# Robotics-Engineer-khy/ti5_isaacgym

Measured on AMD Instinct MI355X. Metric: env-steps/sec at 8192 envs, t1_dh_stand, 1/2/4/8 MI355X; obs/reward parity, higher is better.
Workload: dtype f32

## Files before the change

### ti5_isaacgym_amd/csrc/t1env_device.h

```cpp
#pragma once
#include <hip/hip_runtime.h>

#include "../../include/t1env.h"
#include "t1_dynamics.h"

namespace t1 {

struct DevWriter {
  float* rootp;
  float* rigidp;
  float* contactp;
  __device__ void root(const float* v) {
#pragma unroll
    for (int i = 0; i < 13; ++i) rootp[i] = v[i];
  }
  __device__ void rigid(int b, const float* v) {
#pragma unroll
    for (int i = 0; i < 13; ++i) rigidp[b * 13 + i] = v[i];
  }
  __device__ void contact(int b, V3<float> f) {
    contactp[b * 3 + 0] = f.x;
    contactp[b * 3 + 1] = f.y;
    contactp[b * 3 + 2] = f.z;
  }
// ... 349 lines not shown
        store16B<SC1>(out0 + i, o);
        continue;
      }
      const uint32_t ow[4] = {o.x, o.y, o.z, o.w};
#pragma unroll
      for (int k = 0; k < 8; ++k) {
        const uint32_t e = i + k;
        if (e >= lim) break;
        if (e - (e / ROW) * ROW < ROW - F) store2B<SC1>(out0 + e, (uint16_t)(ow[k / 2] >> (16 * (k & 1))));
      }
    }
  }
}

__device__ __forceinline__ void shift_history(const ShiftArgs& S, int64_t t0, int64_t stride) {
  if (S.half) {
    shift_range_h<T1_NOBS, T1_HIST>(reinterpret_cast<const uint16_t*>(S.obs_in), reinterpret_cast<uint16_t*>(S.obs_out),
                                    S.total_obs, 0, (S.total_obs + 7) / 8, t0, stride);
    shift_range_h<T1_NPRIV, T1_CHIST>(reinterpret_cast<const uint16_t*>(S.priv_in),
                                      reinterpret_cast<uint16_t*>(S.priv_out), S.total_priv, 0, (S.total_priv + 7) / 8,
                                      t0, stride);
    return;
  }
  shift_range<T1_NOBS, T1_HIST>(S.obs_in, S.obs_out, S.total_obs, 0, (S.total_obs + 3) / 4, t0, stride);
  shift_range<T1_NPRIV, T1_CHIST>(S.priv_in, S.priv_out, S.total_priv, 0, (S.total_priv + 3) / 4, t0, stride);
}

template <int U = SHIFT_UNROLL>
__device__ __forceinline__ void shift_rows_range_sc1(const ShiftArgs& S, int64_t r0, int64_t r1, int64_t t0,
                                                 int64_t stride) {
  if (S.half) {
    shift_rows_f16<T1_NOBS, T1_HIST, true, U>(reinterpret_cast<const uint16_t*>(S.obs_in),
                                              reinterpret_cast<uint16_t*>(S.obs_out), S.total_obs, r0, r1, (int)t0,
                                              (int)stride);
    shift_rows_f16<T1_NPRIV, T1_CHIST, true, U>(reinterpret_cast<const uint16_t*>(S.priv_in),
                                                reinterpret_cast<uint16_t*>(S.priv_out), S.total_priv, r0, r1, (int)t0,
                                                (int)stride);
    return;
  }
  shift_rows_f32<T1_NOBS, T1_HIST, true, U>(S.obs_in, S.obs_out, S.total_obs, r0, r1, (int)t0, (int)stride);
  shift_rows_f32<T1_NPRIV, T1_CHIST, true, U>(S.priv_in, S.priv_out, S.total_priv, r0, r1, (int)t0, (int)stride);
}

__device__ __forceinline__ void zero_hist(float* buf, bool half, int64_t row, int width, int count, int t0, int stride) {
  if (half) {
    uint16_t* o = reinterpret_cast<uint16_t*>(buf) + row * width;
    for (int c = t0; c < count; c += stride) o[c] = 0;
  } else {
    float* o = buf + row * width;
    for (int c = t0; c < count; c += stride) o[c] = 0.0f;
  }
}

__device__ __forceinline__ void zero_history_row(const ShiftArgs& S, int64_t row, int t0, int stride) {
  zero_hist(S.obs_out, S.half, row, T1_NOBS * T1_HIST, T1_NOBS * (T1_HIST - 1), t0, stride);
  zero_hist(S.priv_out, S.half, row, T1_NPRIV * T1_CHIST, T1_NPRIV * (T1_CHIST - 1), t0, stride);
}

}
```

### ti5_isaacgym_amd/csrc/t1env_dyn6.hip

```cpp
#include <hip/hip_runtime.h>

#define T1_CONTACT_ONE_COPY

#ifdef T1_PROBE_SIMD
__device__ unsigned g_t1_simd6[4096][8];
#endif
#ifdef T1_PROBE_CLOCK
__device__ unsigned long long g_t1_clock6[4];
constexpr int T1_WGSUM6_N = 4 + 6;
__device__ unsigned long long g_t1_wgtime6[4096][4];
__device__ unsigned long long g_t1_wgsum6[4096][T1_WGSUM6_N];
#define T1_CLOCK_WAIT_BEGIN() const unsigned long long t1c_w0 = __builtin_amdgcn_s_memtime();
#define T1_CLOCK_SHIFT_END(wi)                                                     \
  if ((threadIdx.x & 63) == 0 && blockIdx.x < 4096 && (wi) >= 0)                   \
    atomicAdd(&g_t1_wgsum6[blockIdx.x][4 + (wi)], __builtin_amdgcn_s_memtime() - t1c_w0);
#define T1_CLOCK_LOOP_END()                                                        \
  if (threadIdx.x == 0 && blockIdx.x < 4096) g_t1_wgtime6[blockIdx.x][3] = __builtin_amdgcn_s_memrealtime();
#define T1_CLOCK_WAIT_END(k)                                                       \
  if (threadIdx.x == 0 && blockIdx.x < 4096)                                       \
    atomicAdd(&g_t1_wgsum6[blockIdx.x][k], __builtin_amdgcn_s_memtime() - t1c_w0);
#define T1_CLOCK_BEGIN()                                                           \
  unsigned long long t1c_cyc0 = 0, t1c_rt0 = 0;                                    \
  if (threadIdx.x == 0) {                                                          \
    t1c_cyc0 = __builtin_amdgcn_s_memtime();                                       \
    t1c_rt0 = __builtin_amdgcn_s_memrealtime();                                    \
    if (blockIdx.x < 4096) { g_t1_wgtime6[blockIdx.x][0] = t1c_rt0; g_t1_wgtime6[blockIdx.x][2] = 0; } \
  }
#define T1_CLOCK_END()                                                             \
  if (threadIdx.x == 0) {                                                          \
    const unsigned long long c1 = __builtin_amdgcn_s_memtime(), r1 = __builtin_amdgcn_s_memrealtime(); \
    atomicAdd(&g_t1_clock6[0], c1 - t1c_cyc0);                                     \
    atomicAdd(&g_t1_clock6[1], r1 - t1c_rt0);                                      \
    atomicAdd(&g_t1_clock6[2], 1ull);                                              \
    if (blockIdx.x < 4096) {                                                       \
      g_t1_wgtime6[blockIdx.x][1] = r1;                                            \
      atomicAdd(&g_t1_wgsum6[blockIdx.x][0], c1 - t1c_cyc0);                       \
    }                                                                              \
  }                                                                                \
  T1_CLOCK_WAVE_END();
#define T1_CLOCK_WAVE_END()                                                        \
  if ((threadIdx.x & 63) == 0 && blockIdx.x < 4096)                                \
    atomicMax(&g_t1_wgtime6[blockIdx.x][2], (unsigned long long)__builtin_amdgcn_s_memrealtime());
#else
#define T1_CLOCK_BEGIN() ((void)0)
#define T1_CLOCK_END() ((void)0)
#define T1_CLOCK_WAVE_END() ((void)0)
#define T1_CLOCK_WAIT_BEGIN() ((void)0)
#define T1_CLOCK_WAIT_END(k) ((void)0)
#define T1_CLOCK_SHIFT_END(wi) ((void)0)
#define T1_CLOCK_LOOP_END() ((void)0)
#endif

#define T1_PROF_WAVES 8
#define T1_PROF_NAME(x) x##6
#include "t1env_prof.h"

#include "t1_dyn5.h"
#include "t1env_device.h"
#include "t1env_internal.h"
#include "t1env_postphys.h"
#include "t1env_fused.h"
#include "t1env_roles.h"

using namespace t1;

constexpr int NE6 = 32;
constexpr int D6_BLOCK = 512;

enum : int { WB_TAU = 0, WB_AC = 8, WB_R = 29, WB_N = 35 };
struct SubspaceRows { float4 r[NLEG][2][64]; };
enum : int { R_RG = 0, R_G = 6, R_N = 12 };
enum : int { WC_SHA = 0, WC_SHB = 1, WC_FTA = 2, WC_FTB = 3, WC_SSH = 4, WC_SFT = 5, WC_N = 6 };
constexpr int SHIFT6_MASK = (1 << 1) | (1 << 5) | (1 << 2) | (1 << 6) | (1 << 3) | (1 << 7);
__device__ __forceinline__ int role_of(int wave) { return (int)((0x76543210u >> (4 * wave)) & 0xFu); }
constexpr int SHIFT6_WAVES = __builtin_popcount(SHIFT6_MASK);
static_assert((SHIFT6_MASK & 0x11) == 0, "W0 / W4 (the core chain's SIMD) do not shift");

struct Dyn6Lds {
  DynModel model;
  Rows4<Q_N> st;
  Rows4<WB_N> wb;
  SubspaceRows sj;
  Rows4<R_N> w1;
  Rows4<XCH> wc[WC_N];
  PdStage<64> pd;
  float cap[CAP5_N][64];
  float act[12][NE6];
  float epi[EPI_N][NE6];
  float fr[FR_N][NE6];
  float vish[64];
  float vift[64];
  float amx[4][64];
  LegParams<float> pl[64];
  BaseParams<float> pb[64];
  float rtf[2][3][64];
  float rsf[2][3][64];
};
T1_ROWS_ALIGNED(Dyn6Lds, st);
T1_ROWS_ALIGNED(Dyn6Lds, wb);
T1_ROWS_ALIGNED(Dyn6Lds, sj);
T1_ROWS_ALIGNED(Dyn6Lds, w1);
T1_ROWS_ALIGNED(Dyn6Lds, wc);
static_assert(sizeof(Rows4<XCH>) % 16 == 0 && alignof(Dyn6Lds) % 16 == 0, "every wc[i], and the struct itself");

template <int F, int H, bool HALF>
__device__ __forceinline__ void shift_chunk_elems(const uint8_t* in0, uint8_t* out0, uint32_t i, uint32_t nel) {
  constexpr uint32_t ROW = F * H, PER = HALF ? 8 : 4;
#pragma unroll 1
  for (uint32_t k = 0; k < PER; ++k) {
    const uint32_t e = i + k;
    if (e < nel && e % ROW < ROW - F) {
      if constexpr (HALF)
        reinterpret_cast<uint16_t*>(out0)[e] = reinterpret_cast<const uint16_t*>(in0)[e + F];
      else
        reinterpret_cast<float*>(out0)[e] = reinterpret_cast<const float*>(in0)[e + F];
    }
  }
}
template <int F, int H, bool HALF>
__device__ __forceinline__ void shp_range(int64_t total, int64_t r0, int64_t r1, int sl, int nsl, uint32_t& lo,
                                          uint32_t& hi, uint32_t& lim, uint32_t& nel) {
  constexpr uint32_t ROW = F * H, PER = HALF ? 8 : 4;
  lim = (uint32_t)(total - r0 * (int64_t)ROW);
  const uint32_t span = (uint32_t)((r1 - r0) * ROW);
  nel = span < lim ? span : lim;
  const uint32_t n = (nel + PER - 1) / PER;
  lo = n * (uint32_t)sl / (uint32_t)nsl;
  hi = n * (uint32_t)(sl + 1) / (uint32_t)nsl;
}
typedef float shift_f4 __attribute__((ext_vector_type(4), aligned(2)));
template <int F, bool HALF, int U>
__device__ __forceinline__ void shift_loads(const uint8_t* in0, uint32_t lo, uint32_t lim, int t0, int stride,
                                            float4* a) {
  constexpr uint32_t PER = HALF ? 8 : 4, ES = HALF ? 2 : 4;
#pragma unroll
  for (int u = 0; u < U; ++u) {
    const uint32_t src = (lo + (uint32_t)(t0 + u * stride)) * PER + F;
    const uint32_t sc = src + PER <= lim ? src : lim - PER;
    const shift_f4 v = *reinterpret_cast<const shift_f4*>(in0 + (size_t)sc * ES);
    a[u] = make_float4(v.x, v.y, v.z, v.w);
  }
}
template <int F, int H, bool HALF, int U>
__device__ __forceinline__ void shift_stores(const uint8_t* in0, uint8_t* out0, uint32_t lo, uint32_t hi,
                                             uint32_t lim, uint32_t nel, int t0, int stride, const float4* a) {
  constexpr uint32_t PER = HALF ? 8 : 4, ES = HALF ? 2 : 4;
  uint32_t slow = 0;
#pragma unroll
  for (int u = 0; u < U; ++u) {
// ... 644 lines not shown
          }
        } else {
          const int s = role == 2 ? 0 : 1;
          const int b = s == 0 ? bsh : bft;
          const float vt = restitution_target(M, eg, s == 0 ? lds.vish[lane] : lds.vift[lane]);
          const V3<float> f = body_contact_force(M, T, b, Ko[s].Rb, Ko[s].p, F.abs, Ko[s].V, mu, vt);
          lds.rtf[s][0][lane] = f.x; lds.rtf[s][1][lane] = f.y; lds.rtf[s][2][lane] = f.z;
        }
      }
      T1_PROF_MARK(10);
      if (role == 6) {
        const int s_dof = (nsub - 1) - B.dof_lag_timestep[n] % 10;
        const int s_imu = (nsub - 1) - B.imu_lag_timestep[n] % 10;
        BaseState<float> sb;
        float q[NLEG], qd[NLEG];
        read_state_rows(lds.st, lane, sb, q, qd);
        record_substep(M, lds.pb[lane], LG, lds, nsub - 1, s_dof, s_imu, N, n, j0, leg, lane, active, sb, q, qd);
        if (active) {
          float* const dof_dst = B.dof_hist + ((size_t)n * 4 + (ctr & 3u)) * 24;
          float* const imu_dst = B.imu_hist + ((size_t)n * 2 + (ctr & 1u)) * 8;
          if (s_dof < nsub) {
#pragma unroll
            for (int k = 0; k < NLEG; ++k) {
              dof_dst[j0 + k] = lds.cap[k][lane];
              dof_dst[12 + j0 + k] = lds.cap[NLEG + k][lane];
            }
          }
          if (leg == 0 && s_imu < nsub) {
            const float quat[4] = {lds.cap[2 * NLEG][lane], lds.cap[2 * NLEG + 1][lane], lds.cap[2 * NLEG + 2][lane],
                                   lds.cap[2 * NLEG + 3][lane]};
            const float w[3] = {lds.cap[2 * NLEG + 4][lane], lds.cap[2 * NLEG + 5][lane], lds.cap[2 * NLEG + 6][lane]};
            capture_imu(quat, w, imu_dst);
          }
        }
      }
      __syncthreads();
      T1_PROF_MARK(11);
      if (role == 6) {
        float* cf = B.contact_forces + (size_t)n * 39;
#pragma unroll
        for (int s = 0; s < 2; ++s) {
          const int b = s == 0 ? bsh : bft;
          const float f[3] = {lds.rtf[s][0][lane] + lds.rsf[s][0][lane], lds.rtf[s][1][lane] + lds.rsf[s][1][lane],
                              lds.rtf[s][2][lane] + lds.rsf[s][2][lane]};
          if (active) { cf[b * 3 + 0] = f[0]; cf[b * 3 + 1] = f[1]; cf[b * 3 + 2] = f[2]; }
          if (FUSED && s == 1) {
            const int r = leg == 0 ? F_C0 : F_C1;
            lds.fr[r][e] = f[0]; lds.fr[r + 1][e] = f[1]; lds.fr[r + 2][e] = f[2];
          }
        }
      }
    }
    if constexpr (FUSED) {
      __syncthreads();
      T1_PROF_MARK(12);
      if (role == 1)
        fused_epilogue_staged<POST_A_STATE, NE6, true>(M, C, B, A, S, FA, dyn_blocks, lane, lds.epi, lds.fr, lds.act,
                                                       lds.act + NLEG);
      else if (role == 2)
        fused_epilogue_obs<POST_OBS_PRIV, NE6>(M, C, B, A, lane, lds.epi, lds.fr, lds.act, lds.act + NLEG);
      else if (role == 3)
        fused_epilogue_obs<POST_OBS_ACTOR, NE6>(M, C, B, A, lane, lds.epi, lds.fr, lds.act, lds.act + NLEG);
      T1_PROF_MARK(15);
    }
    T1_CLOCK_WAVE_END();
    T1_PROF_END();
    return;
  }

  BaseParams<float>& PB = lds.pb[lane];
  LegParams<float>& PL = lds.pl[lane];
  {
    BaseState<float> sb;
    float q[NLEG], qd[NLEG];
    BaseParams<float> pb;
    LegParams<float> pl;
    load_base_params(M, B, n, pb);
    load_leg_params(M, B, n, j0, pl);
    load_base_state(M, pb, B.root_states + (size_t)n * 13, sb);
    PB = pb;
    PL = pl;
#pragma unroll
    for (int k = 0; k < NLEG; ++k) {
      q[k] = B.dof_state[n * 24 + 2 * (j0 + k)];
      qd[k] = B.dof_state[n * 24 + 2 * (j0 + k) + 1];
    }
    float v[Q_N];
    state_pack(sb, q, qd, v);
    put4(lds.st, lane, v);
  }
  float vi_ft = B.contact_vimp[(size_t)n * NVIMP + vimp_foot(leg)];
  float vi_sh = B.contact_vimp[(size_t)n * NVIMP + vimp_shank(leg)];
  lds.vift[lane] = vi_ft;
  lds.vish[lane] = vi_sh;
  T1_PROF_MARK(0);
  for (int sub = 0; sub < nsub; ++sub) {
    {
      T1_CLOCK_WAIT_BEGIN();
      __syncthreads();
      T1_CLOCK_WAIT_END(sub == 0 ? 3 : 1);
    }
    T1_PROF_MARK(1);
    const DynModel& M = model_in_loop(lds.model);
    LegBlock<float> lb;
    Sym6<float> Ab;
    {
      BaseState<float> sb;
      float q[NLEG], qd[NLEG];
      {
        float v[Q_N];
        get4w(lds.st, lane, v);
        state_unpack(v, sb, q, qd);
      }
      const M3<float> R0 = quat_to_mat(sb.quat[0], sb.quat[1], sb.quat[2], sb.quat[3]);
      LegFK<float> fk;
// ... 60 lines not shown
      r[i] = (r[i] + l) + rr;
    }
    Prod<float> r0;
    solve_base<true>(Ac, r, &r0);
    float dq[NLEG];
    backsub_leg<true>(lb, r, dq);
    BaseState<float> sb;
    float q[NLEG], qd[NLEG];
    read_state_rows<true>(lds.st, lane, sb, q, qd);
    integrate_base<true>(sb, r, dt, &r0);
    integrate_leg<true>(M, leg, q, qd, dq, dt);
    float v[Q_N];
    state_pack(sb, q, qd, v);
    put4w(lds.st, lane, v);
    T1_PROF_MARK(7);
  }
  T1_CLOCK_LOOP_END();
  BaseState<float> sb;
  float q[NLEG], qd[NLEG];
  read_state_rows<true>(lds.st, lane, sb, q, qd);
  int no = n;
  asm volatile("" : "+v"(no));
  if (active) {
    B.contact_vimp[(size_t)no * NVIMP + vimp_foot(leg)] = vi_ft;
    B.contact_vimp[(size_t)no * NVIMP + vimp_shank(leg)] = vi_sh;
#pragma unroll
    for (int k = 0; k < NLEG; ++k) {
      B.dof_state[no * 24 + 2 * (j0 + k)] = q[k];
      B.dof_state[no * 24 + 2 * (j0 + k) + 1] = qd[k];
    }
  }
  float (*FR)[NE6] = FUSED ? lds.fr : nullptr;
  if constexpr (FUSED) {
#pragma unroll
    for (int k = 0; k < NLEG; ++k) {
      lds.fr[F_DOF + 2 * (j0 + k)][e] = q[k];
      lds.fr[F_DOF + 2 * (j0 + k) + 1][e] = qd[k];
    }
  }
  T1_PROF_MARK(8);
  __syncthreads();
  T1_PROF_MARK(9);
  {
    BaseFrame<float> F;
    base_frame(sb, F);
    leg_report_rigid<NE6>(M, B, PB, sb, F, q, qd, no, leg, active, e, FR);
  }
  T1_PROF_MARK(10);
  __syncthreads();
  T1_PROF_MARK(11);
  if constexpr (FUSED) {
    __syncthreads();
    T1_PROF_MARK(12);
    fused_epilogue_staged<POST_A_REWARDS, NE6, true>(M, C, B, A, S, FA, dyn_blocks, lane, lds.epi, lds.fr, lds.act,
                                                     lds.act + NLEG);
  }
  T1_CLOCK_END();
  T1_PROF_END();
}

#ifdef T1_PROBE_SIMD
extern "C" int t1env_debug_simd6(unsigned* out, int blocks) {
  return (int)hipMemcpyFromSymbol(out, HIP_SYMBOL(g_t1_simd6), sizeof(unsigned) * 8 * (size_t)blocks);
}
#endif

#ifdef T1_PROBE_CLOCK
extern "C" int t1env_debug_wgtime6(unsigned long long* out, int blocks) {
  return (int)hipMemcpyFromSymbol(out, HIP_SYMBOL(g_t1_wgtime6), sizeof(unsigned long long) * 4 * (size_t)blocks);
}
extern "C" int t1env_debug_wgsum6(unsigned long long* out, int blocks, int reset) {
  hipError_t e = hipMemcpyFromSymbol(out, HIP_SYMBOL(g_t1_wgsum6), sizeof(unsigned long long) * T1_WGSUM6_N * (size_t)blocks);
  if (e == hipSuccess && reset) {
    static unsigned long long zero[4096][T1_WGSUM6_N] = {};
    e = hipMemcpyToSymbol(HIP_SYMBOL(g_t1_wgsum6), zero, sizeof(zero));
  }
  return (int)e;
}
extern "C" int t1env_debug_clock6(unsigned long long* out, int reset) {
  hipError_t e = hipMemcpyFromSymbol(out, HIP_SYMBOL(g_t1_clock6), sizeof(g_t1_clock6));
  if (e == hipSuccess && reset) {
    static const unsigned long long zero[4] = {};
    e = hipMemcpyToSymbol(HIP_SYMBOL(g_t1_clock6), zero, sizeof(zero));
  }
  return (int)e;
}
#endif

int t1_launch_dyn6(const DynModel* d_model, const t1env_config* d_cfg, const t1env_buffers& B, const Terrain& T,
                   const float* actions, const t1env_step_args& A, int num_envs, const ShiftArgs& S,
                   const FusedArgs* fused, hipStream_t s, const SubLog* log) {
  const int blocks = (num_envs + NE6 - 1) / NE6;
  const FusedArgs FA = fused ? *fused : FusedArgs{};
  const SubLog LG = log ? *log : SubLog{};
  const bool hf = T.type != 0;
  if (log && !fused) return (int)hipErrorInvalidValue;
#define T1_LAUNCH6(HF, FU) \
  hipLaunchKernelGGL((k_dyn6<HF, FU>), dim3(blocks), dim3(D6_BLOCK), 0, s, d_model, d_cfg, B, T, actions, A, S, blocks, FA, LG)
  if (fused) { if (hf) T1_LAUNCH6(true, true); else T1_LAUNCH6(false, true); }
  else { if (hf) T1_LAUNCH6(true, false); else T1_LAUNCH6(false, false); }
#undef T1_LAUNCH6
  return (int)hipGetLastError();
}
```

### ti5_isaacgym_amd/csrc/t1env_fused.h

```cpp
#pragma once
#include "t1env_device.h"
#include "t1env_internal.h"
#include "t1env_postphys.h"

namespace t1 {

constexpr int SHIFT_UNIT = 8;
constexpr int K_SHANK = 3, K_FOOT = 5;
static_assert(T1_LEG_CONTACT_MASK == ((1 << K_SHANK) | (1 << K_FOOT)), "the step kernels assume shank + foot contacts");
constexpr int XCH = 27;

constexpr uint32_t HANDOFF_SHIFT = 1u, HANDOFF_DYN = 2u;
__device__ __forceinline__ uint32_t unit_handoff(uint32_t* word, uint32_t epoch, uint32_t bits) {
  const uint32_t tag = (epoch & 0x3fffffu) << 10;
  uint32_t old = __hip_atomic_load(word, __ATOMIC_RELAXED, __HIP_MEMORY_SCOPE_AGENT);
  for (;;) {
    const uint32_t nw = ((old & ~0x3ffu) == tag ? old : tag) | bits;
    if (__hip_atomic_compare_exchange_strong(word, &old, nw, __ATOMIC_RELAXED, __ATOMIC_RELAXED,
                                             __HIP_MEMORY_SCOPE_AGENT))
      return nw;
  }
}
__device__ __forceinline__ bool handoff_complete(uint32_t w) { return (w & 3u) == 3u; }

__device__ __forceinline__ void zero_unit_resets(const ShiftArgs& S, int u, uint32_t word, int t0, int stride) {
  uint32_t bits = (word >> 2) & 0xffu;
  while (bits) {
    const int r = __ffs(bits) - 1;
    bits &= bits - 1;
    zero_history_row(S, (int64_t)u * SHIFT_UNIT + r, t0, stride);
  }
}

template <int NE, bool INWG>
__device__ __forceinline__ void epilogue_handoff(const t1env_config& C, const ShiftArgs& S, const FusedArgs& FA, int lane,
                                                 bool do_reset, bool active) {
  const int N = C.num_envs;
  const unsigned long long m = __ballot(do_reset && active);
  if (INWG || FA.shift_done) {
    unsigned long long todo = m;
    while (todo) {
      const int l = __ffsll(todo) - 1;
      todo &= todo - 1;
      zero_history_row(S, (int64_t)blockIdx.x * NE + l, lane, 64);
    }
    return;
  }
  const int units = (N + SHIFT_UNIT - 1) / SHIFT_UNIT;
  const int u = blockIdx.x * (NE / SHIFT_UNIT) + lane;
  uint32_t w = 0;
  if (lane < NE / SHIFT_UNIT && u < units)
    w = unit_handoff(FA.unit_state + u, FA.epoch, HANDOFF_DYN | ((uint32_t)(m >> (lane * SHIFT_UNIT)) & 0xffu) << 2);
  uint64_t todo = __ballot(handoff_complete(w));
  while (todo) {
    const int l = __ffsll((unsigned long long)todo) - 1;
    todo &= todo - 1;
// ... 142 lines not shown
  stage_ld<NE, NT, 3>(B.ext_forces, nb, nv, t, V.ef);
  stage_ld<NE, NT, 3>(B.ext_torques, nb, nv, t, V.et);
  stage_ld<NE, NT, 3>(B.gait_time, nb, nv, t, V.gt);
  stage_ld<NE, NT, 2>(reinterpret_cast<const uint32_t*>(B.episode_length_buf), nb, nv, t, V.el);
  stage_ld<NE, NT, 2>(reinterpret_cast<const uint32_t*>(B.phase_length_buf), nb, nv, t, V.pl);
  stage_ld<NE, NT, 1>(B.gait_start, nb, nv, t, V.gs);
  stage_ld<NE, NT, 2>(B.last_contacts, nb, nv, t, V.lc);
  stage_ld<NE, NT, 1>(B.friction, nb, nv, t, V.fr);
  stage_ld<NE, NT, 1>(B.body_mass, nb, nv, t, V.ms);
  stage_ld<NE, NT, 1>(B.dof_lag_timestep, nb, nv, t, V.dl);
  stage_ld<NE, NT, 1>(B.imu_lag_timestep, nb, nv, t, V.il);
#pragma unroll
  for (int i = 0; i < EpiStage<NE, NT>::NES; ++i) {
    const int e = t + NT * i, ec = e < T1_NREW * nv ? e : T1_NREW * nv - 1;
    V.es[i] = B.episode_sums[(size_t)(ec / nv) * N + nb + ec % nv];
  }
}
template <int NE, int NT>
__device__ __forceinline__ void epi_stage_store(int N, int nb, int t, const EpiStage<NE, NT>& V, float (*E)[NE]) {
  const int nv = N - nb < NE ? N - nb : NE;
  stage_st<NE, NT, 12>(E + E_LA, nv, t, V.la);
  stage_st<NE, NT, 12>(E + E_LLA, nv, t, V.lla);
  stage_st<NE, NT, 6>(E + E_LRV, nv, t, V.lrv);
  stage_st<NE, NT, 12>(E + E_LDV, nv, t, V.ldv);
  stage_st<NE, NT, 12>(E + E_REF, nv, t, V.ref);
  stage_st<NE, NT, 4>(E + E_CMD, nv, t, V.cmd);
  stage_st<NE, NT, 2>(E + E_AT, nv, t, V.at);
  stage_st<NE, NT, 2>(E + E_FH, nv, t, V.fh);
  stage_st<NE, NT, 2>(E + E_LFZ, nv, t, V.lfz);
  stage_st<NE, NT, 3>(E + E_EF, nv, t, V.ef);
  stage_st<NE, NT, 3>(E + E_ET, nv, t, V.et);
  stage_st<NE, NT, 3>(E + E_GT, nv, t, V.gt);
  stage_st<NE, NT, 2>(E + E_EL, nv, t, V.el);
  stage_st<NE, NT, 2>(E + E_PL, nv, t, V.pl);
  stage_st<NE, NT, 1>(E + E_GS, nv, t, V.gs);
  stage_st<NE, NT, 2>(E + E_LC, nv, t, V.lc);
  stage_st<NE, NT, 1>(E + E_FRIC, nv, t, V.fr);
  stage_st<NE, NT, 1>(E + E_MASS, nv, t, V.ms);
  stage_st<NE, NT, 1>(E + E_DL, nv, t, V.dl);
  stage_st<NE, NT, 1>(E + E_IL, nv, t, V.il);
#pragma unroll
  for (int i = 0; i < EpiStage<NE, NT>::NES; ++i) {
    const int e = t + NT * i, ec = e < T1_NREW * nv ? e : T1_NREW * nv - 1;
    E[E_ESUM + ec / nv][ec % nv] = V.es[i];
  }
}
template <int NE, int NT>
__device__ __forceinline__ void stage_epilogue_inputs(const t1env_buffers& B, int N, int nb, int t, float (*E)[NE]) {
  EpiStage<NE, NT> V;
  epi_stage_load<NE, NT>(B, N, nb, t, V);
  epi_stage_store<NE, NT>(N, nb, t, V, E);
}

template <int PART, int NE, bool INWG>
__device__ __forceinline__ void fused_epilogue_staged(const DynModel& M, const t1env_config& C, const t1env_buffers& B,
                                                      const t1env_step_args& A, const ShiftArgs& S,
                                                      const FusedArgs& FA, int dyn_blocks, int lane,
                                                      const float (*E)[NE], const float (*FR)[NE],
                                                      const float (*ACT0)[NE], const float (*ACT1)[NE]) {
  const int N = C.num_envs;
  const int e = lane % NE;
  const int n0 = lane < NE ? (int)blockIdx.x * NE + lane : N;
  const bool active = n0 < N;
  const int n = active ? n0 : N - 1;
  PostAIn X;
#pragma unroll
  for (int i = 0; i < 13; ++i) X.root[i] = FR[F_ROOT + i][e];
#pragma unroll
  for (int i = 0; i < 24; ++i) X.dof[i] = FR[F_DOF + i][e];
#pragma unroll
  for (int i = 0; i < 13; ++i) { X.f0[i] = FR[F_F0 + i][e]; X.f1[i] = FR[F_F1 + i][e]; }
#pragma unroll
  for (int i = 0; i < 2; ++i) { X.k0[i] = FR[F_K0 + i][e]; X.k1[i] = FR[F_K1 + i][e]; }
#pragma unroll
  for (int i = 0; i < 3; ++i) { X.cfb[i] = FR[F_CFB + i][e]; X.c0[i] = FR[F_C0 + i][e]; X.c1[i] = FR[F_C1 + i][e]; }
#pragma unroll
  for (int i = 0; i < 12; ++i) X.tq[i] = FR[F_TQ + i][e];
#pragma unroll
  for (int k = 0; k < NLEG; ++k) { X.a[k] = ACT0[k][e]; X.a[NLEG + k] = ACT1[k][e]; }
#pragma unroll
  for (int i = 0; i < 12; ++i) {
    X.la[i] = E[E_LA + i][e]; X.lla[i] = E[E_LLA + i][e];
    X.ldv[i] = E[E_LDV + i][e]; X.ref[i] = E[E_REF + i][e];
  }
#pragma unroll
  for (int i = 0; i < 6; ++i) X.lrv[i] = E[E_LRV + i][e];
#pragma unroll
  for (int i = 0; i < 4; ++i) X.cmd[i] = E[E_CMD + i][e];
#pragma unroll
  for (int i = 0; i < 2; ++i) {
    X.at[i] = E[E_AT + i][e]; X.fh[i] = E[E_FH + i][e]; X.lfz[i] = E[E_LFZ + i][e];
    X.lc[i] = (uint8_t)__float_as_int(E[E_LC + i][e]);
  }
#pragma unroll
  for (int i = 0; i < 3; ++i) {
    X.ef[i] = E[E_EF + i][e]; X.et[i] = E[E_ET + i][e];
    X.gt[i] = __float_as_int(E[E_GT + i][e]);
  }
#pragma unroll
  for (int k = 0; k < T1_NREW; ++k) X.esum[k] = E[E_ESUM + k][e];
  X.el = (int64_t)(((uint64_t)(uint32_t)__float_as_int(E[E_EL + 1][e]) << 32) |
                   (uint32_t)__float_as_int(E[E_EL][e]));
  X.pl = (int64_t)(((uint64_t)(uint32_t)__float_as_int(E[E_PL + 1][e]) << 32) |
                   (uint32_t)__float_as_int(E[E_PL][e]));
  X.gstart = E[E_GS][e];
  BaseQ bq;
  float* const ep_row = FA.ep_part + (size_t)blockIdx.x * EP_PART_ROW;
  const bool do_reset = post_a_core<PART>(M, C, B, A, n0, X, bq, PART == POST_A_REWARDS ? ep_row : nullptr);
  T1_PROF_MARK(13);
  if constexpr (PART == POST_A_REWARDS) {
    epilogue_handoff<NE, INWG>(C, S, FA, lane, do_reset, active);
    __builtin_amdgcn_s_waitcnt(0);
    __syncthreads();
    epilogue_finalize_parts(C, B, A, FA, dyn_blocks, lane);
    T1_PROF_MARK(15);
    return;
  }
  if (active && do_reset) {
    const uint32_t genv = (uint32_t)(C.env_offset + n);
    const uint32_t ctr = A.counter + 1u;
    const float pos_cmd[4] = {X.root[0], X.root[1], X.cmd[0], X.cmd[1]};
    reset_env(M, C, B, A, n, genv, ctr, true, false, true, pos_cmd);
    ObsIn O;
#pragma unroll
    for (int i = 0; i < 4; ++i) O.cmd[i] = X.cmd[i];
    reset_obs_inputs(M, C, rng_key(C.seed, genv, ctr), O, false);
    if (resample_commands_r(C, A, O.el, O.gt, O.cmd, genv, ctr)) strow(B.commands + n * 4, O.cmd);
  }
  T1_PROF_MARK(14);
  wave_sum_store(ep_row + T1_ACC_LEVEL, (C.custom_origins && active) ? (float)B.terrain_levels[n] : 0.0f);
  __builtin_amdgcn_s_waitcnt(0);
  __syncthreads();
  T1_PROF_MARK(15);
}

template <int PART, int NE>
__device__ __forceinline__ void fused_epilogue_obs(const DynModel& M, const t1env_config& C, const t1env_buffers& B,
                                                   const t1env_step_args& A, int lane, const float (*E)[NE],
                                                   const float (*FR)[NE], const float (*ACT0)[NE],
                                                   const float (*ACT1)[NE]) {
  static_assert(PART == POST_OBS_PRIV || PART == POST_OBS_ACTOR, "an observation part");
  constexpr bool PRIV = PART == POST_OBS_PRIV;
  const int e = lane % NE;
  const int n = (int)blockIdx.x * NE + lane;
  if (lane >= NE || n >= C.num_envs) return;
  const uint32_t genv = (uint32_t)(C.env_offset + n);
  const uint32_t ctr = A.counter + 1u;
  const RngKey K = rng_key(C.seed, genv, ctr);
  float ld[24], lraw[8];
  if constexpr (!PRIV)
    load_lagged(B, A, n, __float_as_int(E[E_DL][e]), __float_as_int(E[E_IL][e]), ld, lraw);
  ObsIn O;
#pragma unroll
  for (int i = 0; i < 4; ++i) O.cmd[i] = E[E_CMD + i][e];
#pragma unroll
  for (int i = 0; i < 3; ++i) O.gt[i] = __float_as_int(E[E_GT + i][e]);
  const int64_t el = (int64_t)(((uint64_t)(uint32_t)__float_as_int(E[E_EL + 1][e]) << 32) |
                               (uint32_t)__float_as_int(E[E_EL][e])) + 1;
  const int64_t pl = (int64_t)(((uint64_t)(uint32_t)__float_as_int(E[E_PL + 1][e]) << 32) |
                               (uint32_t)__float_as_int(E[E_PL][e])) + 1;
  O.gstart = E[E_GS][e];
#pragma unroll
  for (int i = 0; i < 24; ++i) O.dof[i] = FR[F_DOF + i][e];
#pragma unroll
  for (int k = 0; k < NLEG; ++k) { O.act[k] = ACT0[k][e]; O.act[NLEG + k] = ACT1[k][e]; }
  ObsExtra Ex;
  if constexpr (PRIV) {
    float root[13], ef[3], et[3], af[3];
#pragma unroll
    for (int i = 0; i < 13; ++i) root[i] = FR[F_ROOT + i][e];
#pragma unroll
    for (int i = 0; i < 3; ++i) { ef[i] = E[E_EF + i][e]; et[i] = E[E_ET + i][e]; }
#pragma unroll
    for (int i = 0; i < 12; ++i) O.la[i] = E[E_LA + i][e];
    base_quantities_r(root, O.bq);
    bool ext_store;
    post_callback(C, A, genv, ctr, K, el, O.gt, O.cmd, root, ef, et, af, ext_store);
#pragma unroll
    for (int i = 0; i < 6; ++i) O.rv[i] = root[7 + i];
    Ex.ef[0] = ef[0]; Ex.ef[1] = ef[1];
#pragma unroll
    for (int i = 0; i < 3; ++i) Ex.et[i] = et[i];
    Ex.cfz[0] = FR[F_C0 + 2][e]; Ex.cfz[1] = FR[F_C1 + 2][e];
    Ex.fric = E[E_FRIC][e];
    Ex.mass = E[E_MASS][e];
// ... 118 lines not shown
```

### ti5_isaacgym_amd/csrc/t1env_postphys.h

```cpp
#pragma once
#include "t1env_device.h"

namespace t1 {

struct Phase {
  float sin_pos;
  float stance[2];
};

template <int K, typename T>
__device__ __forceinline__ void ldrow(T (&d)[K], const T* s) {
#pragma unroll
  for (int i = 0; i < K; ++i) d[i] = s[i];
}
template <int K, typename T>
__device__ __forceinline__ void strow(T* d, const T (&s)[K]) {
#pragma unroll
  for (int i = 0; i < K; ++i) d[i] = s[i];
}

__device__ __forceinline__ float phase_value(const t1env_config& C, int64_t phase_len, float gait_start, bool stand) {
  const float dtf = (float)(C.sim_dt * C.decimation);
  float ph = ((float)phase_len * dtf) / C.cycle_time;
  ph = ph - floorf(ph);
// ... 529 lines not shown
}

__device__ __forceinline__ bool post_a_env(const DynModel& M, const t1env_config& C, const t1env_buffers& B,
                                           const t1env_step_args& A, int n0) {
  const int n = n0 < C.num_envs ? n0 : C.num_envs - 1;
  PostAIn X;
  load_post_a_in(B, (size_t)C.num_envs, n, X);
  BaseQ bq;
  return post_a_core(M, C, B, A, n0, X, bq);
}

struct ObsIn {
  float cmd[4], dof[24], act[12], la[12], rv[6];
  BaseQ bq;
  int32_t gt[3];
  int64_t el, pl;
  float gstart;
  int dl, il;
};

__device__ __forceinline__ void reset_obs_inputs(const DynModel& M, const t1env_config& C, RngKey K, ObsIn& X,
                                                 bool dof = true) {
  if (dof)
#pragma unroll
    for (int j = 0; j < 12; ++j) {
      X.dof[2 * j] = M.default_dof_pos[j] + rand_float(-C.reset_dof_range, C.reset_dof_range, K, SLOT_RESET_DOF + j);
      X.dof[2 * j + 1] = 0.0f;
    }
#pragma unroll
  for (int j = 0; j < 12; ++j) { X.act[j] = 0.0f; X.la[j] = 0.0f; }
  float r[13];
#pragma unroll
  for (int i = 0; i < 13; ++i) r[i] = M.base_init_state[i];
#pragma unroll
  for (int i = 0; i < 6; ++i) X.rv[i] = r[7 + i];
  base_quantities_r(r, X.bq);
  X.dl = rand_int(C.dof_lag_range[0], C.dof_lag_range[1] + 1, K, SLOT_LAG_DOF);
  X.il = rand_int(C.imu_lag_range[0], C.imu_lag_range[1] + 1, K, SLOT_LAG_IMU);
  X.gstart = (float)rand_int(0, 2, K, SLOT_GAIT_START) * 0.5f;
  float g[3];
#pragma unroll
  for (int i = 0; i < 3; ++i)
    g[i] = rand_float(C.gait_time_range[i][0], C.gait_time_range[i][1], K, SLOT_GAIT_TIME + i);
  const float gs = (g[0] + g[1]) + g[2];
  const float f = C.max_episode_length / gs;
  const float s0 = g[0] * f, s1 = g[1] * f;
  X.gt[0] = 0;
  X.gt[1] = (int32_t)(0.0f + s0);
  X.gt[2] = (int32_t)((0.0f + s0) + s1);
  X.el = 0;
  X.pl = 0;
}

__device__ __forceinline__ void reset_env(const DynModel& M, const t1env_config& C, const t1env_buffers& B, const t1env_step_args& A,
                          int n, uint32_t genv, uint32_t ctr, bool do_terrain, bool zero_reward_state = true,
                          bool obs_elsewhere = false, const float* pos_cmd = nullptr) {
  const RngKey K = rng_key(C.seed, genv, ctr);
  float org[3];
  bool org_known = false;
  if (do_terrain && C.terrain_curriculum) {
    const float* r = pos_cmd ? pos_cmd : B.root_states + n * 13;
    const float* o = B.env_origins + n * 3;
    const float dist = norm2(r[0] - o[0], r[1] - o[1]);
    const bool up = dist > C.env_length / 2.0f;
    const float* cmd = pos_cmd ? pos_cmd + 2 : B.commands + n * 4;
    const bool down = (dist < norm2(cmd[0], cmd[1]) * (C.episode_length_s * 0.5f)) && !up;
    int lv = B.terrain_levels[n] + (up ? 1 : 0) - (down ? 1 : 0);
    const int rnd = rand_int(0, C.num_terrain_rows, K, SLOT_TERRAIN_LEVEL_RAND);
    lv = lv >= C.num_terrain_rows ? rnd : (lv < 0 ? 0 : lv);
    B.terrain_levels[n] = lv;
    const float* to = B.terrain_origins + ((size_t)lv * C.num_terrain_cols + B.terrain_types[n]) * 3;
#pragma unroll
    for (int i = 0; i < 3; ++i) {
      org[i] = to[i];
      B.env_origins[n * 3 + i] = org[i];
    }
    org_known = true;
  }
  if (!org_known)
#pragma unroll
    for (int i = 0; i < 3; ++i) org[i] = B.env_origins[n * 3 + i];
  ObsIn R;
  reset_obs_inputs(M, C, K, R);
#pragma unroll
  for (int i = 0; i < NVIMP; ++i) B.contact_vimp[(size_t)n * NVIMP + i] = 0.0f;
#pragma unroll
  for (int j = 0; j < 24; ++j) B.dof_state[n * 24 + j] = R.dof[j];
  float r[13];
#pragma unroll
  for (int i = 0; i < 13; ++i) r[i] = M.base_init_state[i];
#pragma unroll
  for (int i = 0; i < 3; ++i) r[i] += org[i];
  if (C.custom_origins) {
    const float p3 = C.reset_xy_range;
    r[0] += rand_float(-p3, p3, K, SLOT_RESET_ROOT_XY + 0);
    r[1] += rand_float(-p3, p3, K, SLOT_RESET_ROOT_XY + 1);
  }
  strow(B.root_states + n * 13, r);
#pragma unroll
  for (int j = 0; j < 12; ++j) {
    B.motor_offsets[n * 12 + j] =
        rand_float(C.motor_offset_range[0], C.motor_offset_range[1], K, SLOT_DR_OFFSET + j);
    B.kp[n * 12 + j] = rand_float(C.kp_mult_range[0], C.kp_mult_range[1], K, SLOT_DR_KP + j) * M.p_gains[j];
    B.kd[n * 12 + j] = rand_float(C.kd_mult_range[0], C.kd_mult_range[1], K, SLOT_DR_KD + j) * M.d_gains[j];
    B.coulomb[n * 12 + j] = rand_float(C.coulomb_range[0], C.coulomb_range[1], K, SLOT_DR_COULOMB + j);
    B.viscous[n * 12 + j] = rand_float(C.viscous_range[0], C.viscous_range[1], K, SLOT_DR_VISCOUS + j);
    B.armature[n * 12 + j] = rand_float(C.armature_range[j][0], C.armature_range[j][1], K,
                                        SLOT_DR_ARMATURE + (C.armature_shared ? 0 : j));
  }
#pragma unroll
  for (int i = 0; i < 48; ++i) B.act_hist[(size_t)n * 48 + i] = 0.0f;
#pragma unroll
  for (int i = 0; i < 96; ++i) B.dof_hist[(size_t)n * 96 + i] = 0.0f;
#pragma unroll
  for (int i = 0; i < 16; ++i) B.imu_hist[(size_t)n * 16 + i] = 0.0f;
  B.lag_timestep[n] = rand_int(C.lag_range[0], C.lag_range[1] + 1, K, SLOT_LAG_ACTION);
  B.dof_lag_timestep[n] = R.dl;
  B.imu_lag_timestep[n] = R.il;
#pragma unroll
  for (int j = 0; j < 12; ++j) B.actions[n * 12 + j] = 0.0f;
  if (!obs_elsewhere) {
#pragma unroll
    for (int j = 0; j < 12; ++j) {
      B.last_last_actions[n * 12 + j] = 0.0f;
      B.last_actions[n * 12 + j] = 0.0f;
      B.last_dof_vel[n * 12 + j] = 0.0f;
    }
#pragma unroll
    for (int i = 0; i < 6; ++i) B.last_root_vel[n * 6 + i] = 0.0f;
  }
  if (zero_reward_state) {
    B.feet_air_time[n * 2 + 0] = 0.0f;
    B.feet_air_time[n * 2 + 1] = 0.0f;
  }
  B.episode_length_buf[n] = 0;
  B.phase_length_buf[n] = 0;
  B.reset_buf[n] = 1;
  B.gait_start[n] = R.gstart;
  strow(B.gait_time + n * 3, R.gt);
  if (zero_reward_state)
#pragma unroll
    for (int k = 0; k < T1_NREW; ++k) B.episode_sums[(size_t)k * C.num_envs + n] = 0.0f;
  store_base_quantities(B, n, R.bq);
}

__device__ __forceinline__ float obs_noise(const t1env_config& C, RngKey K, int i) {
  const float u = uniform01(K, SLOT_OBS_NOISE + i);
  return ((2.0f * u - 1.0f) * C.noise_vec[i]) * C.noise_level;
}

__device__ __forceinline__ void load_obs_in(const t1env_buffers& B, int n, ObsIn& X) {
  ldrow(X.cmd, B.commands + n * 4);
  ldrow(X.dof, B.dof_state + (size_t)n * 24);
  ldrow(X.act, B.actions + n * 12);
  ldrow(X.la, B.last_actions + n * 12);
  const float* r = B.root_states + n * 13;
#pragma unroll
  for (int i = 0; i < 6; ++i) X.rv[i] = r[7 + i];
  ldrow(X.bq.lin, B.base_lin_vel + n * 3);
  ldrow(X.bq.ang, B.base_ang_vel + n * 3);
  ldrow(X.bq.euler, B.base_euler_xyz + n * 3);
  ldrow(X.gt, B.gait_time + n * 3);
  X.el = B.episode_length_buf[n];
  X.pl = B.phase_length_buf[n];
  X.gstart = B.gait_start[n];
  X.dl = B.dof_lag_timestep[n];
  X.il = B.imu_lag_timestep[n];
}

struct ObsExtra {
  float ef[2], et[3], cfz[2], fric, mass;
};
__device__ __forceinline__ void post_b_core(const DynModel& M, const t1env_config& C, const t1env_buffers& B,
                                            const t1env_step_args& A, int n, bool do_reset, bool any_reset, ObsIn& X,
                                            const ObsExtra& E, bool zero_reward_state = true);
__device__ __forceinline__ void post_b_env(const DynModel& M, const t1env_config& C, const t1env_buffers& B,
                                           const t1env_step_args& A, int n, bool do_reset, bool any_reset) {
  ObsIn X;
  load_obs_in(B, n, X);
  ObsExtra E;
  ldrow(E.ef, B.ext_forces + n * 3);
  ldrow(E.et, B.ext_torques + n * 3);
  E.cfz[0] = B.contact_forces[(size_t)n * 39 + 6 * 3 + 2];
  E.cfz[1] = B.contact_forces[(size_t)n * 39 + 12 * 3 + 2];
  E.fric = B.friction[n];
  E.mass = B.body_mass[n];
  post_b_core(M, C, B, A, n, do_reset, any_reset, X, E);
}

struct ObsPhase {
  float sp, cp, ref[12];
  Phase ph;
};
__device__ __forceinline__ void obs_phase(const DynModel& M, const t1env_config& C, const ObsIn& X, bool stand,
                                          ObsPhase& P) {
  const float phase = phase_value(C, X.pl, X.gstart, stand);
// ... 172 lines not shown
```

Before: 71.84 million.

## Overlap reset work with reward epilogue via LDS flag, offload row zeroing to idle waves

```diff
diff --git a/ti5_isaacgym_amd/csrc/t1env_device.h b/ti5_isaacgym_amd/csrc/t1env_device.h
--- a/ti5_isaacgym_amd/csrc/t1env_device.h
+++ b/ti5_isaacgym_amd/csrc/t1env_device.h
@@ -425,9 +425,27 @@
   }
 }
 
+template <typename T>
+__device__ __forceinline__ void zero_span_wide(T* o, int count, int t0, int stride) {
+  typedef uint32_t u32x4 __attribute__((ext_vector_type(4)));
+  const uintptr_t a = reinterpret_cast<uintptr_t>(o), b = a + (uintptr_t)count * sizeof(T);
+  uintptr_t a16 = (a + 15) & ~(uintptr_t)15, b16 = b & ~(uintptr_t)15;
+  if (a16 > b16) a16 = b16 = b;
+  const int head = (int)((a16 - a) / sizeof(T)), mid = (int)((b16 - a16) / 16), tail = (int)((b - b16) / sizeof(T));
+  u32x4* const m = reinterpret_cast<u32x4*>(a16);
+  for (int c = t0; c < mid; c += stride) m[c] = u32x4{0u, 0u, 0u, 0u};
+  for (int c = t0; c < head; c += stride) o[c] = (T)0;
+  T* const t = reinterpret_cast<T*>(b16);
+  for (int c = t0; c < tail; c += stride) t[c] = (T)0;
+}
+__device__ __forceinline__ void zero_hist_wide(float* buf, bool half, int64_t row, int width, int count, int t0, int stride) {
+  if (half) zero_span_wide(reinterpret_cast<uint16_t*>(buf) + row * width, count, t0, stride);
+  else zero_span_wide(buf + row * width, count, t0, stride);
+}
+
 __device__ __forceinline__ void zero_history_row(const ShiftArgs& S, int64_t row, int t0, int stride) {
-  zero_hist(S.obs_out, S.half, row, T1_NOBS * T1_HIST, T1_NOBS * (T1_HIST - 1), t0, stride);
-  zero_hist(S.priv_out, S.half, row, T1_NPRIV * T1_CHIST, T1_NPRIV * (T1_CHIST - 1), t0, stride);
-}
-
-}
+  zero_hist_wide(S.obs_out, S.half, row, T1_NOBS * T1_HIST, T1_NOBS * (T1_HIST - 1), t0, stride);
+  zero_hist_wide(S.priv_out, S.half, row, T1_NPRIV * T1_CHIST, T1_NPRIV * (T1_CHIST - 1), t0, stride);
+}
+
+}
diff --git a/ti5_isaacgym_amd/csrc/t1env_dyn6.hip b/ti5_isaacgym_amd/csrc/t1env_dyn6.hip
--- a/ti5_isaacgym_amd/csrc/t1env_dyn6.hip
+++ b/ti5_isaacgym_amd/csrc/t1env_dyn6.hip
@@ -41,6 +41,11 @@
 #define T1_CLOCK_WAVE_END()                                                        \
   if ((threadIdx.x & 63) == 0 && blockIdx.x < 4096)                                \
     atomicMax(&g_t1_wgtime6[blockIdx.x][2], (unsigned long long)__builtin_amdgcn_s_memrealtime());
+constexpr int T1_TAIL6_N = 16;
+__device__ unsigned long long g_t1_tail6[4096][T1_TAIL6_N];
+#define T1_CLOCK_STAMP(k)                                                          \
+  if ((threadIdx.x & 63) == 0 && blockIdx.x < 4096)                                \
+    g_t1_tail6[blockIdx.x][k] = __builtin_amdgcn_s_memrealtime();
 #else
 #define T1_CLOCK_BEGIN() ((void)0)
 #define T1_CLOCK_END() ((void)0)
@@ -49,6 +54,7 @@
 #define T1_CLOCK_WAIT_END(k) ((void)0)
 #define T1_CLOCK_SHIFT_END(wi) ((void)0)
 #define T1_CLOCK_LOOP_END() ((void)0)
+#define T1_CLOCK_STAMP(k) ((void)0)
 #endif
 
 #define T1_PROF_WAVES 8
@@ -95,6 +101,7 @@
   BaseParams<float> pb[64];
   float rtf[2][3][64];
   float rsf[2][3][64];
+  uint32_t e2;
 };
 T1_ROWS_ALIGNED(Dyn6Lds, st);
 T1_ROWS_ALIGNED(Dyn6Lds, wb);
@@ -845,15 +852,18 @@
       }
     }
     if constexpr (FUSED) {
+      if (role == 1 && lane == 0) lds.e2 = 0u;
       __syncthreads();
       T1_PROF_MARK(12);
       if (role == 1)
-        fused_epilogue_staged<POST_A_STATE, NE6, true>(M, C, B, A, S, FA, dyn_blocks, lane, lds.epi, lds.fr, lds.act,
-                                                       lds.act + NLEG);
+        fused_epilogue_staged<POST_A_STATE, NE6, true, false>(M, C, B, A, S, FA, dyn_blocks, lane, lds.epi,
+                                                                             lds.fr, lds.act, lds.act + NLEG, &lds.e2);
       else if (role == 2)
         fused_epilogue_obs<POST_OBS_PRIV, NE6>(M, C, B, A, lane, lds.epi, lds.fr, lds.act, lds.act + NLEG);
       else if (role == 3)
         fused_epilogue_obs<POST_OBS_ACTOR, NE6>(M, C, B, A, lane, lds.epi, lds.fr, lds.act, lds.act + NLEG);
+      else if (wave >= 5)
+        epilogue_zero_reset_rows<NE6>(C, B, S, lane, (int)threadIdx.x - 320, 192, lds.epi, lds.fr);
       T1_PROF_MARK(15);
     }
     T1_CLOCK_WAVE_END();
@@ -1020,8 +1030,8 @@
   if constexpr (FUSED) {
     __syncthreads();
     T1_PROF_MARK(12);
-    fused_epilogue_staged<POST_A_REWARDS, NE6, true>(M, C, B, A, S, FA, dyn_blocks, lane, lds.epi, lds.fr, lds.act,
-                                                     lds.act + NLEG);
+    fused_epilogue_staged<POST_A_REWARDS, NE6, true, false>(M, C, B, A, S, FA, dyn_blocks, lane, lds.epi,
+                                                                           lds.fr, lds.act, lds.act + NLEG, &lds.e2);
   }
   T1_CLOCK_END();
   T1_PROF_END();
@@ -1036,6 +1046,9 @@
 #ifdef T1_PROBE_CLOCK
 extern "C" int t1env_debug_wgtime6(unsigned long long* out, int blocks) {
   return (int)hipMemcpyFromSymbol(out, HIP_SYMBOL(g_t1_wgtime6), sizeof(unsigned long long) * 4 * (size_t)blocks);
+}
+extern "C" int t1env_debug_tail6(unsigned long long* out, int blocks) {
+  return (int)hipMemcpyFromSymbol(out, HIP_SYMBOL(g_t1_tail6), sizeof(unsigned long long) * T1_TAIL6_N * (size_t)blocks);
 }
 extern "C" int t1env_debug_wgsum6(unsigned long long* out, int blocks, int reset) {
   hipError_t e = hipMemcpyFromSymbol(out, HIP_SYMBOL(g_t1_wgsum6), sizeof(unsigned long long) * T1_WGSUM6_N * (size_t)blocks);
diff --git a/ti5_isaacgym_amd/csrc/t1env_fused.h b/ti5_isaacgym_amd/csrc/t1env_fused.h
--- a/ti5_isaacgym_amd/csrc/t1env_fused.h
+++ b/ti5_isaacgym_amd/csrc/t1env_fused.h
@@ -2,6 +2,10 @@
 #include "t1env_device.h"
 #include "t1env_internal.h"
 #include "t1env_postphys.h"
+
+#ifndef T1_CLOCK_STAMP
+#define T1_CLOCK_STAMP(k) ((void)0)
+#endif
 
 namespace t1 {
 
@@ -250,13 +254,50 @@
   epi_stage_store<NE, NT>(N, nb, t, V, E);
 }
 
-template <int PART, int NE, bool INWG>
+template <int NE>
+__device__ __forceinline__ void epilogue_zero_reset_rows(const t1env_config& C, const t1env_buffers& B,
+                                                         const ShiftArgs& S, int lane, int t, int nt,
+                                                         const float (*E)[NE], const float (*FR)[NE]) {
+  const int e = lane % NE;
+  const int n = (int)blockIdx.x * NE + lane;
+  const int64_t el = (int64_t)(((uint64_t)(uint32_t)__float_as_int(E[E_EL + 1][e]) << 32) |
+                               (uint32_t)__float_as_int(E[E_EL][e])) + 1;
+  const bool term = norm3(FR[F_CFB][e], FR[F_CFB + 1][e], FR[F_CFB + 2][e]) > 1.0f;
+  const bool tout = (float)el > C.max_episode_length;
+  unsigned long long todo = __ballot(lane < NE && n < C.num_envs && (term || tout));
+  while (todo) {
+    const int l = __ffsll(todo) - 1;
+    todo &= todo - 1;
+    const int64_t row = (int64_t)blockIdx.x * NE + l;
+    zero_history_row(S, row, t, nt);
+    zero_span_wide(B.act_hist + row * 48, 48, t, nt);
+    zero_span_wide(B.dof_hist + row * 96, 96, t, nt);
+    zero_span_wide(B.imu_hist + row * 16, 16, t, nt);
+  }
+}
+
+__device__ __forceinline__ void epilogue_reset_rest(const DynModel& M, const t1env_config& C, const t1env_buffers& B,
+                                                    const t1env_step_args& A, int n, uint32_t genv, uint32_t ctr,
+                                                    RngKey K, const float (&cmd)[4], float org[3], bool org_known,
+                                                    bool zero_lag_rings) {
+  reset_env_rest(M, C, B, n, K, org, org_known, false, true, zero_lag_rings);
+  ObsIn O;
+#pragma unroll
+  for (int i = 0; i < 4; ++i) O.cmd[i] = cmd[i];
+  reset_obs_inputs(M, C, K, O, false);
+  if (resample_commands_r(C, A, O.el, O.gt, O.cmd, genv, ctr)) strow(B.commands + n * 4, O.cmd);
+}
+
+template <int PART, int NE, bool INWG, bool RESET_ROWS = true>
 __device__ __forceinline__ void fused_epilogue_staged(const DynModel& M, const t1env_config& C, const t1env_buffers& B,
                                                       const t1env_step_args& A, const ShiftArgs& S,
                                                       const FusedArgs& FA, int dyn_blocks, int lane,
                                                       const float (*E)[NE], const float (*FR)[NE],
-                                                      const float (*ACT0)[NE], const float (*ACT1)[NE]) {
+                                                      const float (*ACT0)[NE], const float (*ACT1)[NE],
+                                                      uint32_t* e2_flag = nullptr) {
   const int N = C.num_envs;
+  constexpr int TS = PART == POST_A_REWARDS ? 0 : 8;
+  T1_CLOCK_STAMP(TS);
   const int e = lane % NE;
   const int n0 = lane < NE ? (int)blockIdx.x * NE + lane : N;
   const bool active = n0 < N;
@@ -304,31 +345,52 @@
   X.gstart = E[E_GS][e];
   BaseQ bq;
   float* const ep_row = FA.ep_part + (size_t)blockIdx.x * EP_PART_ROW;
+  const bool in_level_sum = PART == POST_A_STATE && C.custom_origins && active;
+  int level = in_level_sum ? B.terrain_levels[n] : 0;
   const bool do_reset = post_a_core<PART>(M, C, B, A, n0, X, bq, PART == POST_A_REWARDS ? ep_row : nullptr);
   T1_PROF_MARK(13);
+  T1_CLOCK_STAMP(TS + 1);
   if constexpr (PART == POST_A_REWARDS) {
-    epilogue_handoff<NE, INWG>(C, S, FA, lane, do_reset, active);
+    if constexpr (RESET_ROWS) epilogue_handoff<NE, INWG>(C, S, FA, lane, do_reset, active);
+    T1_CLOCK_STAMP(TS + 2);
     __builtin_amdgcn_s_waitcnt(0);
-    __syncthreads();
+    T1_CLOCK_STAMP(TS + 3);
+    if (e2_flag) {
+      while (__hip_atomic_load(e2_flag, __ATOMIC_ACQUIRE, __HIP_MEMORY_SCOPE_WORKGROUP) == 0u) __builtin_amdgcn_s_sleep(1);
+    } else {
+      __syncthreads();
+    }
+    T1_CLOCK_STAMP(TS + 4);
     epilogue_finalize_parts(C, B, A, FA, dyn_blocks, lane);
+    T1_CLOCK_STAMP(TS + 5);
     T1_PROF_MARK(15);
     return;
   }
+  const uint32_t genv = (uint32_t)(C.env_offset + n);
+  const uint32_t ctr = A.counter + 1u;
+  const RngKey K = rng_key(C.seed, genv, ctr);
+  float org[3];
+  bool org_known = false;
   if (active && do_reset) {
-    const uint32_t genv = (uint32_t)(C.env_offset + n);
-    const uint32_t ctr = A.counter + 1u;
     const float pos_cmd[4] = {X.root[0], X.root[1], X.cmd[0], X.cmd[1]};
-    reset_env(M, C, B, A, n, genv, ctr, true, false, true, pos_cmd);
-    ObsIn O;
-#pragma unroll
-    for (int i = 0; i < 4; ++i) O.cmd[i] = X.cmd[i];
-    reset_obs_inputs(M, C, rng_key(C.seed, genv, ctr), O, false);
-    if (resample_commands_r(C, A, O.el, O.gt, O.cmd, genv, ctr)) strow(B.commands + n * 4, O.cmd);
-  }
+    org_known = reset_curriculum(C, B, n, K, true, pos_cmd, org, level, in_level_sum);
+  }
+  if (!e2_flag && active && do_reset)
+    epilogue_reset_rest(M, C, B, A, n, genv, ctr, K, X.cmd, org, org_known, RESET_ROWS);
   T1_PROF_MARK(14);
-  wave_sum_store(ep_row + T1_ACC_LEVEL, (C.custom_origins && active) ? (float)B.terrain_levels[n] : 0.0f);
+  T1_CLOCK_STAMP(TS + 2);
+  wave_sum_store(ep_row + T1_ACC_LEVEL, in_level_sum ? (float)level : 0.0f);
   __builtin_amdgcn_s_waitcnt(0);
-  __syncthreads();
+  T1_CLOCK_STAMP(TS + 3);
+  if (e2_flag) {
+    if (lane == 0) __hip_atomic_store(e2_flag, 1u, __ATOMIC_RELEASE, __HIP_MEMORY_SCOPE_WORKGROUP);
+  } else {
+    __syncthreads();
+  }
+  T1_CLOCK_STAMP(TS + 4);
+  if (e2_flag && active && do_reset)
+    epilogue_reset_rest(M, C, B, A, n, genv, ctr, K, X.cmd, org, org_known, RESET_ROWS);
+  T1_CLOCK_STAMP(TS + 5);
   T1_PROF_MARK(15);
 }
 
diff --git a/ti5_isaacgym_amd/csrc/t1env_postphys.h b/ti5_isaacgym_amd/csrc/t1env_postphys.h
--- a/ti5_isaacgym_amd/csrc/t1env_postphys.h
+++ b/ti5_isaacgym_amd/csrc/t1env_postphys.h
@@ -605,31 +605,34 @@
   X.pl = 0;
 }
 
-__device__ __forceinline__ void reset_env(const DynModel& M, const t1env_config& C, const t1env_buffers& B, const t1env_step_args& A,
-                          int n, uint32_t genv, uint32_t ctr, bool do_terrain, bool zero_reward_state = true,
-                          bool obs_elsewhere = false, const float* pos_cmd = nullptr) {
-  const RngKey K = rng_key(C.seed, genv, ctr);
-  float org[3];
-  bool org_known = false;
-  if (do_terrain && C.terrain_curriculum) {
-    const float* r = pos_cmd ? pos_cmd : B.root_states + n * 13;
-    const float* o = B.env_origins + n * 3;
-    const float dist = norm2(r[0] - o[0], r[1] - o[1]);
-    const bool up = dist > C.env_length / 2.0f;
-    const float* cmd = pos_cmd ? pos_cmd + 2 : B.commands + n * 4;
-    const bool down = (dist < norm2(cmd[0], cmd[1]) * (C.episode_length_s * 0.5f)) && !up;
-    int lv = B.terrain_levels[n] + (up ? 1 : 0) - (down ? 1 : 0);
-    const int rnd = rand_int(0, C.num_terrain_rows, K, SLOT_TERRAIN_LEVEL_RAND);
-    lv = lv >= C.num_terrain_rows ? rnd : (lv < 0 ? 0 : lv);
-    B.terrain_levels[n] = lv;
-    const float* to = B.terrain_origins + ((size_t)lv * C.num_terrain_cols + B.terrain_types[n]) * 3;
-#pragma unroll
-    for (int i = 0; i < 3; ++i) {
-      org[i] = to[i];
-      B.env_origins[n * 3 + i] = org[i];
-    }
-    org_known = true;
-  }
+__device__ __forceinline__ bool reset_curriculum(const t1env_config& C, const t1env_buffers& B, int n, RngKey K,
+                                                 bool do_terrain, const float* pos_cmd, float org[3], int& lv_io,
+                                                 bool lv_known = false) {
+  if (!(do_terrain && C.terrain_curriculum)) return false;
+  const float* r = pos_cmd ? pos_cmd : B.root_states + n * 13;
+  const float* o = B.env_origins + n * 3;
+  const float dist = norm2(r[0] - o[0], r[1] - o[1]);
+  const bool up = dist > C.env_length / 2.0f;
+  const float* cmd = pos_cmd ? pos_cmd + 2 : B.commands + n * 4;
+  const bool down = (dist < norm2(cmd[0], cmd[1]) * (C.episode_length_s * 0.5f)) && !up;
+  int lv = (lv_known ? lv_io : B.terrain_levels[n]) + (up ? 1 : 0) - (down ? 1 : 0);
+  const int rnd = rand_int(0, C.num_terrain_rows, K, SLOT_TERRAIN_LEVEL_RAND);
+  lv = lv >= C.num_terrain_rows ? rnd : (lv < 0 ? 0 : lv);
+  B.terrain_levels[n] = lv;
+  const float* to = B.terrain_origins + ((size_t)lv * C.num_terrain_cols + B.terrain_types[n]) * 3;
+#pragma unroll
+  for (int i = 0; i < 3; ++i) {
+    org[i] = to[i];
+    B.env_origins[n * 3 + i] = org[i];
+  }
+  lv_io = lv;
+  return true;
+}
+
+__device__ __forceinline__ void reset_env_rest(const DynModel& M, const t1env_config& C, const t1env_buffers& B,
+                                               int n, RngKey K, float org[3], bool org_known,
+                                               bool zero_reward_state = true, bool obs_elsewhere = false,
+                                               bool zero_lag_rings = true) {
   if (!org_known)
 #pragma unroll
     for (int i = 0; i < 3; ++i) org[i] = B.env_origins[n * 3 + i];
@@ -661,12 +664,14 @@
     B.armature[n * 12 + j] = rand_float(C.armature_range[j][0], C.armature_range[j][1], K,
                                         SLOT_DR_ARMATURE + (C.armature_shared ? 0 : j));
   }
-#pragma unroll
-  for (int i = 0; i < 48; ++i) B.act_hist[(size_t)n * 48 + i] = 0.0f;
-#pragma unroll
-  for (int i = 0; i < 96; ++i) B.dof_hist[(size_t)n * 96 + i] = 0.0f;
-#pragma unroll
-  for (int i = 0; i < 16; ++i) B.imu_hist[(size_t)n * 16 + i] = 0.0f;
+  if (zero_lag_rings) {
+#pragma unroll
+    for (int i = 0; i < 48; ++i) B.act_hist[(size_t)n * 48 + i] = 0.0f;
+#pragma unroll
+    for (int i = 0; i < 96; ++i) B.dof_hist[(size_t)n * 96 + i] = 0.0f;
+#pragma unroll
+    for (int i = 0; i < 16; ++i) B.imu_hist[(size_t)n * 16 + i] = 0.0f;
+  }
   B.lag_timestep[n] = rand_int(C.lag_range[0], C.lag_range[1] + 1, K, SLOT_LAG_ACTION);
   B.dof_lag_timestep[n] = R.dl;
   B.imu_lag_timestep[n] = R.il;
@@ -695,6 +700,16 @@
 #pragma unroll
     for (int k = 0; k < T1_NREW; ++k) B.episode_sums[(size_t)k * C.num_envs + n] = 0.0f;
   store_base_quantities(B, n, R.bq);
+}
+
+__device__ __forceinline__ void reset_env(const DynModel& M, const t1env_config& C, const t1env_buffers& B, const t1env_step_args& A,
+                          int n, uint32_t genv, uint32_t ctr, bool do_terrain, bool zero_reward_state = true,
+                          bool obs_elsewhere = false, const float* pos_cmd = nullptr) {
+  const RngKey K = rng_key(C.seed, genv, ctr);
+  float org[3];
+  int lv;
+  const bool org_known = reset_curriculum(C, B, n, K, do_terrain, pos_cmd, org, lv);
+  reset_env_rest(M, C, B, n, K, org, org_known, zero_reward_state, obs_elsewhere);
 }
 
 __device__ __forceinline__ float obs_noise(const t1env_config& C, RngKey K, int i) {
```

After: 72.99 million (median of 6 runs). +1.6%, better.
